# automl/TransformersCanDoBayesianInference

Hardware: NVIDIA H100
Metric: prior-sampled sequences/sec, full training step (prior sample + fwd + bwd + allreduce + clip + Adam) (higher is better)
Workload: dtype bf16

## Files before the change

### transformerscandobayesianinference_b200/csrc/attention_bwd_tc.cu

```cuda
#include "attention_common.cuh"

namespace pfn {

constexpr int AB_ROWS = 64;
constexpr int AB_TILE = AB_ROWS * ATT_ROW_BYTES;
constexpr int AB_THREADS = 3 * 128;
constexpr int AB_DQ_STAGES = 4;
constexpr int AB_DKV_STAGES = 3;
constexpr int AB_DQ_OFF_RING = 4 * AB_TILE;
constexpr int AB_DQ_OFF_BAR = AB_DQ_OFF_RING + AB_DQ_STAGES * 2 * AB_TILE;
constexpr int AB_DQ_SMEM = AB_DQ_OFF_BAR + (2 * AB_DQ_STAGES + 2) * 8 + 1024;
constexpr int AB_DKV_OFF_RING = 4 * AB_TILE;
constexpr int AB_DKV_OFF_STAT = AB_DKV_OFF_RING + AB_DKV_STAGES * 2 * AB_TILE;
constexpr int AB_DKV_OFF_BAR = AB_DKV_OFF_STAT + AB_DKV_STAGES * 2 * AB_ROWS * 4;
constexpr int AB_DKV_SMEM = AB_DKV_OFF_BAR + (2 * AB_DKV_STAGES + 1) * 8 + 1024;
static_assert(AB_DQ_SMEM <= 232448 && AB_DKV_SMEM <= 232448, "the tiles and rings must fit the 227 KB of shared memory");

struct AttnBwdParams {
  int T, B, H, sep;
  float scale, scale_log2;
  const __nv_bfloat16* qkv; int ld_qkv;
  const __nv_bfloat16* dout; int ld_dout;
  __nv_bfloat16* dqkv; int ld_dqkv;
  const float* lse;
  const float* delta;
  int delta_tm;
  float* dq_colsum;
  uint32_t drop_seed; int drop_thr;
  int n_tiles;
  int batch_major;
};

__device__ __forceinline__ float ab_delta(const AttnBwdParams& p, int b, int h, int i) {
  return p.delta_tm ? p.delta[att_tok(i, b, p.T, p.B, 0) * p.H + h] : p.delta[(static_cast<size_t>(b) * p.H + h) * p.T + i];
}

__device__ __forceinline__ uint64_t ab_desc_k(uint32_t tile, int kk) {
  return tc::wgmma_smem_desc(tile + (kk >> 2) * 8192 + (kk & 3) * 32, 16, 1024);
}
__device__ __forceinline__ uint64_t ab_desc_mn(uint32_t tile, int kk) {
  return tc::wgmma_smem_desc(tile + kk * 2048, 8192, 1024);
}
__device__ __forceinline__ uint32_t ab_opaque(uint32_t addr) {
  asm volatile("" : "+r"(addr));
  return addr;
}
__device__ __forceinline__ void ab_mma_n64(float (&d)[32], uint64_t a_desc, uint64_t b_desc, int kk) {
  if (kk == 0) tc::wgmma_m64n64k16<0>(d, a_desc, b_desc);
  else tc::wgmma_m64n64k16<1>(d, a_desc, b_desc);
}

__device__ __forceinline__ void ab_load_tile(uint8_t* dst, const CUtensorMap* m, uint64_t* bar, int col0, int b, int t0) {
  tc::tma_load_3d(dst, m, bar, col0, b, t0);
  tc::tma_load_3d(dst + 8192, m, bar, col0 + 64, b, t0);
}

__global__ void __launch_bounds__(256)
attn_bwd_delta_kernel(const __nv_bfloat16* __restrict__ out, int ld_out, const __nv_bfloat16* __restrict__ dout,
                      int ld_dout, float* __restrict__ delta, int T, int B, int H, int batch_major) {
  const int lane = threadIdx.x & 31;
  const long long warp = (static_cast<long long>(blockIdx.x) * blockDim.x + threadIdx.x) >> 5;
  const long long nwarps = (static_cast<long long>(gridDim.x) * blockDim.x) >> 5;
  const long long rows = static_cast<long long>(T) * B;
  for (long long tok = warp; tok < rows; tok += nwarps) {
    const int t = batch_major ? static_cast<int>(tok % T) : static_cast<int>(tok / B);
    const int b = batch_major ? static_cast<int>(tok / T) : static_cast<int>(tok % B);
    for (int h0 = 0; h0 < H; h0 += 2) {
      const int h = h0 + (lane >> 4);
      float acc = 0.f;
      if (h < H) {
        const int col = h * ATT_DH + (lane & 15) * 8;
        const uint4 pa = *reinterpret_cast<const uint4*>(out + tok * ld_out + col);
        const uint4 pb = *reinterpret_cast<const uint4*>(dout + tok * ld_dout + col);
        const __nv_bfloat162* ha = reinterpret_cast<const __nv_bfloat162*>(&pa);
        const __nv_bfloat162* hb = reinterpret_cast<const __nv_bfloat162*>(&pb);
#pragma unroll
        for (int j = 0; j < 4; ++j) {
// ... 337 lines not shown
    tc::wgmma_commit();
    tc::wgmma_wait<0>();
    if (tid == 0) tc::mbar_arrive(&empty[stage]);
    if (++stage == AB_DKV_STAGES) { stage = 0; phase ^= 1; }
  }
  tc::wgmma_fence_regs(dk);
  tc::wgmma_fence_regs(dv);

#pragma unroll
  for (int r = 0; r < 2; ++r) {
    const int key = key_a + 8 * r;
    if (key < p.sep) {
      __nv_bfloat16* grow = p.dqkv + att_tok(key, b, p.T, p.B, p.batch_major) * p.ld_dqkv + h * ATT_DH;
#pragma unroll
      for (int j = 0; j < 16; ++j) {
        att_st2(grow + E, j, lane, dk[4 * j + 2 * r], dk[4 * j + 2 * r + 1]);
        att_st2(grow + 2 * E, j, lane, dv[4 * j + 2 * r], dv[4 * j + 2 * r + 1]);
      }
    }
  }
  if (timed_out) asm volatile("trap;");
}

static int ab_tensor_map(CUtensorMap* m, const void* base, int cols, int ld, int T, int B, int t_extent, int batch_major) {
  const uint64_t row = static_cast<uint64_t>(ld) * 2;
  const uint64_t dims[3] = {static_cast<uint64_t>(cols), static_cast<uint64_t>(B), static_cast<uint64_t>(t_extent)};
  const uint64_t strides[3] = {0, batch_major ? row * T : row, batch_major ? row : row * B};
  const uint32_t box[3] = {64, 1, AB_ROWS};
  return make_tensor_map(m, base, false, 3, dims, strides, box, true);
}

}

using namespace pfn;

extern "C" int pfn_attention_bwd_tc(const pfn_attn_desc* d, void* stream) {
  if (int rc = check_tc_attn(d, true, "attention_bwd_tc")) return rc;
  PFN_CHECK_ARG(!(d->delta_token_major && d->batch_major), "attention_bwd_tc: a token-major delta implies the reference token order");
  AttnBwdParams p;
  p.T = d->T; p.B = d->B; p.H = d->H; p.sep = d->sep;
  p.scale = d->scale; p.scale_log2 = d->scale * 1.4426950408889634f;
  p.qkv = reinterpret_cast<const __nv_bfloat16*>(d->qkv); p.ld_qkv = d->ld_qkv;
  p.dout = reinterpret_cast<const __nv_bfloat16*>(d->dout); p.ld_dout = d->ld_dout;
  p.dqkv = reinterpret_cast<__nv_bfloat16*>(d->dqkv); p.ld_dqkv = d->ld_dqkv;
  p.lse = d->lse; p.delta = d->delta; p.dq_colsum = d->dq_colsum; p.delta_tm = d->delta_token_major;
  p.drop_seed = d->drop_seed; p.drop_thr = d->drop_thr;
  p.batch_major = d->batch_major;
  const int E = d->H * ATT_DH;
  CUtensorMap tmQ, tmKV, tmDO;
  if (int rc = ab_tensor_map(&tmQ, d->qkv, 3 * E, d->ld_qkv, d->T, d->B, d->T, d->batch_major)) return rc;
  if (int rc = ab_tensor_map(&tmKV, d->qkv, 3 * E, d->ld_qkv, d->T, d->B, d->sep > 0 ? d->sep : 1, d->batch_major)) return rc;
  if (int rc = ab_tensor_map(&tmDO, d->dout, E, d->ld_dout, d->T, d->B, d->T, d->batch_major)) return rc;
  static bool attr_set[64] = {};
  if (first_use_on_device(attr_set)) {
// ... 27 lines not shown
```

### transformerscandobayesianinference_b200/csrc/attention_common.cuh

```cuda
#pragma once
#include "common.cuh"
#include "dropout.cuh"
#include "tc_common.cuh"
#include "../../include/pfn_b200.h"

namespace pfn {

constexpr int ATT_DH = 128;
constexpr int ATT_ROW_BYTES = ATT_DH * 2;

int check_attn_desc_public(const pfn_attn_desc* d, bool bwd, const char* who);

__device__ __forceinline__ uint32_t att_sw(int r, int c) {
  return static_cast<uint32_t>(r * ATT_ROW_BYTES + ((((c >> 3) ^ (r & 7))) << 4) + (c & 7) * 2);
}

__device__ __forceinline__ size_t att_tok(int t, int b, int T, int B, int batch_major) {
  return batch_major ? static_cast<size_t>(b) * T + t : static_cast<size_t>(t) * B + b;
}

template <int NROWS>
__device__ __forceinline__ void att_load_tile(uint8_t* tile, const __nv_bfloat16* base, int ld, int col0, int t0, int t_end,
                                              int b, int T, int B, int batch_major) {
  const uint32_t s = tc::smem_u32(tile);
#pragma unroll
  for (int k = 0; k < NROWS * 16 / 128; ++k) {
    const int idx = static_cast<int>(threadIdx.x) + 128 * k;
    const int r = idx >> 4, c = idx & 15;
    const int t = t0 + r;
    const bool ok = t < t_end;
    const __nv_bfloat16* src = ok ? base + att_tok(t, b, T, B, batch_major) * ld + col0 + c * 8 : base;
    tc::cp_async16(s + att_sw(r, c * 8), src, ok ? 16u : 0u);
  }
}

__device__ __forceinline__ void att_frag_a(uint32_t (&a)[4], uint32_t tile, int r0, int c0, int lane) {
  tc::ldmatrix_x4(a, tile + att_sw(r0 + (lane & 15), c0 + ((lane >> 4) << 3)));
}
__device__ __forceinline__ void att_frag_b(uint32_t (&b)[4], uint32_t tile, int n0, int k0, int lane) {
  tc::ldmatrix_x4(b, tile + att_sw(n0 + (lane & 7) + ((lane >> 4) << 3), k0 + (((lane >> 3) & 1) << 3)));
}
__device__ __forceinline__ void att_frag_bt(uint32_t (&b)[4], uint32_t tile, int k0, int n0, int lane) {
  tc::ldmatrix_x4_trans(b, tile + att_sw(k0 + (lane & 7) + (((lane >> 3) & 1) << 3), n0 + ((lane >> 4) << 3)));
}

__device__ __forceinline__ float2 att_ld2(const __nv_bfloat16* row, int j, int lane) {
  return __bfloat1622float2(*reinterpret_cast<const __nv_bfloat162*>(row + 8 * j + 2 * (lane & 3)));
}
__device__ __forceinline__ void att_st2(__nv_bfloat16* row, int j, int lane, float x, float y) {
  *reinterpret_cast<uint32_t*>(row + 8 * j + 2 * (lane & 3)) = tc::pack_bf16x2(x, y);
}
__device__ __forceinline__ float quad_sum(float v) {
  v += __shfl_xor_sync(0xffffffffu, v, 1);
  return v + __shfl_xor_sync(0xffffffffu, v, 2);
}
__device__ __forceinline__ float quad_max(float v) {
  v = fmaxf(v, __shfl_xor_sync(0xffffffffu, v, 1));
  return fmaxf(v, __shfl_xor_sync(0xffffffffu, v, 2));
}

static inline int check_tc_attn(const pfn_attn_desc* d, bool bwd, const char* who) {
  if (int rc = check_attn_desc_public(d, bwd, who)) return rc;
  PFN_CHECK_ARG(d->dtype == PFN_BF16, "%s: bf16 only", who);
  PFN_CHECK_ARG(d->dh == ATT_DH, "%s: head dim %d unsupported (built for 128)", who, d->dh);
  PFN_CHECK_ARG(d->ld_qkv % 8 == 0 && d->ld_out % 8 == 0, "%s: leading dims must be multiples of 8", who);
  PFN_CHECK_ARG(((reinterpret_cast<uintptr_t>(d->qkv) | reinterpret_cast<uintptr_t>(d->out)) & 15) == 0,
                "%s: qkv/out must be 16-byte aligned", who);
  if (bwd) {
    PFN_CHECK_ARG(d->ld_dout % 8 == 0 && d->ld_dqkv % 8 == 0, "%s: leading dims must be multiples of 8", who);
    PFN_CHECK_ARG(((reinterpret_cast<uintptr_t>(d->dout) | reinterpret_cast<uintptr_t>(d->dqkv)) & 15) == 0,
                  "%s: dout/dqkv must be 16-byte aligned", who);
  }
  return 0;
}

}
```

### transformerscandobayesianinference_b200/csrc/attention_tc.cu

```cuda
#include "attention_common.cuh"

namespace pfn {

constexpr int ATT_BM = 64;
constexpr int ATT_BN = 64;
constexpr int ATT_TILE_BYTES = ATT_BM * ATT_ROW_BYTES;
constexpr int ATT_FWD_SMEM = 5 * ATT_TILE_BYTES;

struct AttnFwdParams {
  int T, B, H, sep;
  float scale_log2;
  const __nv_bfloat16* qkv; int ld_qkv;
  __nv_bfloat16* out; int ld_out;
  float* lse;
  int n_qtiles;
  int batch_major;
  uint32_t drop_seed; int drop_thr;
};

__global__ void __launch_bounds__(128, 2)
attn_fwd_tc_kernel(const AttnFwdParams p) {
  extern __shared__ __align__(128) uint8_t smem[];
  uint8_t* sQ = smem;
  uint8_t* sK = smem + ATT_TILE_BYTES;
  uint8_t* sV = smem + 3 * ATT_TILE_BYTES;
  const int warp = threadIdx.x >> 5, lane = threadIdx.x & 31;
  const int qt = static_cast<int>(blockIdx.x) % p.n_qtiles;
  const int bh = static_cast<int>(blockIdx.x) / p.n_qtiles;
  const int h = bh % p.H, b = bh / p.H;
  const int E = p.H * ATT_DH;
  const int i0 = qt * ATT_BM;
  const int nblk = (p.sep + ATT_BN - 1) / ATT_BN;

  att_load_tile<ATT_BM>(sQ, p.qkv, p.ld_qkv, h * ATT_DH, i0, p.T, b, p.T, p.B, p.batch_major);
  if (nblk > 0) {
    att_load_tile<ATT_BN>(sK, p.qkv, p.ld_qkv, E + h * ATT_DH, 0, p.sep, b, p.T, p.B, p.batch_major);
    att_load_tile<ATT_BN>(sV, p.qkv, p.ld_qkv, 2 * E + h * ATT_DH, 0, p.sep, b, p.T, p.B, p.batch_major);
  }
  tc::cp_async_commit();

  float o[16][4];
#pragma unroll
  for (int j = 0; j < 16; ++j) o[j][0] = o[j][1] = o[j][2] = o[j][3] = 0.f;
  float m[2] = {-INFINITY, -INFINITY}, l[2] = {0.f, 0.f};
  const int r0 = 16 * warp;
  const uint32_t drow0 = static_cast<uint32_t>(bh) * p.T + i0 + r0 + (lane >> 2);
  const uint32_t q_s = tc::smem_u32(sQ);

  for (int kb = 0; kb < nblk; ++kb) {
    if (kb + 1 < nblk) {
      const int nb = (kb + 1) & 1;
      att_load_tile<ATT_BN>(sK + nb * ATT_TILE_BYTES, p.qkv, p.ld_qkv, E + h * ATT_DH, (kb + 1) * ATT_BN, p.sep, b, p.T, p.B, p.batch_major);
      att_load_tile<ATT_BN>(sV + nb * ATT_TILE_BYTES, p.qkv, p.ld_qkv, 2 * E + h * ATT_DH, (kb + 1) * ATT_BN, p.sep, b, p.T, p.B, p.batch_major);
      tc::cp_async_commit();
      tc::cp_async_wait<1>();
    } else {
      tc::cp_async_wait<0>();
    }
    __syncthreads();
    const uint32_t k_s = tc::smem_u32(sK + (kb & 1) * ATT_TILE_BYTES);
    const uint32_t v_s = tc::smem_u32(sV + (kb & 1) * ATT_TILE_BYTES);

    float s[8][4];
#pragma unroll
    for (int j = 0; j < 8; ++j) s[j][0] = s[j][1] = s[j][2] = s[j][3] = 0.f;
#pragma unroll
    for (int kk = 0; kk < 8; ++kk) {
      uint32_t a[4];
      att_frag_a(a, q_s, r0, kk * 16, lane);
#pragma unroll
      for (int np = 0; np < 4; ++np) {
        uint32_t bb[4];
        att_frag_b(bb, k_s, np * 16, kk * 16, lane);
        tc::mma_bf16_16816(s[2 * np], a, bb[0], bb[1]);
        tc::mma_bf16_16816(s[2 * np + 1], a, bb[2], bb[3]);
      }
    }
    const int key0 = kb * ATT_BN + 2 * (lane & 3);
    float mx[2] = {-INFINITY, -INFINITY};
#pragma unroll
    for (int j = 0; j < 8; ++j)
#pragma unroll
      for (int e = 0; e < 4; ++e) {
        const bool ok = key0 + 8 * j + (e & 1) < p.sep;
        s[j][e] = ok ? s[j][e] * p.scale_log2 : -INFINITY;
        mx[e >> 1] = fmaxf(mx[e >> 1], s[j][e]);
      }
    float corr[2];
#pragma unroll
    for (int r = 0; r < 2; ++r) {
      const float mn = fmaxf(m[r], quad_max(mx[r]));
      corr[r] = fast_ex2(m[r] - mn);
      m[r] = mn;
      l[r] *= corr[r];
    }
#pragma unroll
    for (int j = 0; j < 8; ++j)
#pragma unroll
      for (int e = 0; e < 4; ++e) {
        const float pr = fast_ex2(s[j][e] - m[e >> 1]);
        l[e >> 1] += pr;
        if (p.drop_thr > 0 && !drop_keep(p.drop_seed, drow0 + 8 * (e >> 1), key0 + 8 * j + (e & 1), p.drop_thr)) s[j][e] = 0.f;
        else s[j][e] = pr;
      }
#pragma unroll
    for (int j = 0; j < 16; ++j) {
      o[j][0] *= corr[0]; o[j][1] *= corr[0];
      o[j][2] *= corr[1]; o[j][3] *= corr[1];
    }
#pragma unroll
    for (int kk = 0; kk < 4; ++kk) {
      uint32_t a[4];
      a[0] = tc::pack_bf16x2(s[2 * kk][0], s[2 * kk][1]);
      a[1] = tc::pack_bf16x2(s[2 * kk][2], s[2 * kk][3]);
      a[2] = tc::pack_bf16x2(s[2 * kk + 1][0], s[2 * kk + 1][1]);
      a[3] = tc::pack_bf16x2(s[2 * kk + 1][2], s[2 * kk + 1][3]);
#pragma unroll
      for (int dp = 0; dp < 8; ++dp) {
        uint32_t bb[4];
        att_frag_bt(bb, v_s, kk * 16, dp * 16, lane);
        tc::mma_bf16_16816(o[2 * dp], a, bb[0], bb[1]);
        tc::mma_bf16_16816(o[2 * dp + 1], a, bb[2], bb[3]);
      }
    }
    __syncthreads();
  }

  const float dscale = p.drop_thr > 0 ? drop_scale(p.drop_thr) : 1.0f;
#pragma unroll
  for (int r = 0; r < 2; ++r) {
    const int i = i0 + r0 + (lane >> 2) + 8 * r;
    float lr = quad_sum(l[r]);
    const bool valid = i < p.T;
    const bool diag = valid && i >= p.sep;
    const __nv_bfloat16* qrow = p.qkv + att_tok(valid ? i : 0, b, p.T, p.B, p.batch_major) * p.ld_qkv + h * ATT_DH;
    float sd = 0.f;
    if (diag) {
#pragma unroll
      for (int j = 0; j < 16; ++j) {
        const float2 q = att_ld2(qrow, j, lane), k = att_ld2(qrow + E, j, lane);
        sd = fmaf(q.x, k.x, fmaf(q.y, k.y, sd));
      }
    }
    sd = quad_sum(sd) * p.scale_log2;
    if (diag) {
      const float mn = fmaxf(m[r], sd);
      const float c = fast_ex2(m[r] - mn);
      const float pr = fast_ex2(sd - mn);
      lr = lr * c + pr;
      m[r] = mn;
      const float pd = (p.drop_thr > 0 && !drop_keep(p.drop_seed, drow0 + 8 * r, i, p.drop_thr)) ? 0.f : pr;
#pragma unroll
      for (int j = 0; j < 16; ++j) {
        const float2 v = att_ld2(qrow + 2 * E, j, lane);
        o[j][2 * r] = fmaf(pd, v.x, o[j][2 * r] * c);
        o[j][2 * r + 1] = fmaf(pd, v.y, o[j][2 * r + 1] * c);
      }
    }
    if (valid) {
      const float inv = dscale / lr;
      __nv_bfloat16* orow = p.out + att_tok(i, b, p.T, p.B, p.batch_major) * p.ld_out + h * ATT_DH;
#pragma unroll
      for (int j = 0; j < 16; ++j) att_st2(orow, j, lane, o[j][2 * r] * inv, o[j][2 * r + 1] * inv);
      if ((lane & 3) == 0) p.lse[static_cast<size_t>(bh) * p.T + i] = (m[r] + __log2f(lr)) * 0.69314718055994531f;
    }
  }
}

}

using namespace pfn;

extern "C" int pfn_attention_fwd_tc(const pfn_attn_desc* d, void* stream) {
  if (int rc = check_tc_attn(d, false, "attention_fwd_tc")) return rc;
  AttnFwdParams p;
  p.T = d->T; p.B = d->B; p.H = d->H; p.sep = d->sep;
  p.scale_log2 = d->scale * 1.4426950408889634f;
  p.qkv = reinterpret_cast<const __nv_bfloat16*>(d->qkv); p.ld_qkv = d->ld_qkv;
  p.out = reinterpret_cast<__nv_bfloat16*>(d->out); p.ld_out = d->ld_out;
  p.lse = d->lse;
  p.n_qtiles = (d->T + ATT_BM - 1) / ATT_BM;
  p.batch_major = d->batch_major;
  p.drop_seed = d->drop_seed; p.drop_thr = d->drop_thr;
  const long long grid = static_cast<long long>(p.n_qtiles) * d->B * d->H;
  PFN_CHECK_ARG(grid < (1LL << 31), "attention_fwd_tc: too many tiles");
  static bool attr_set[64] = {};
  if (first_use_on_device(attr_set)) {
    PFN_CUDA_OK(cudaFuncSetAttribute(attn_fwd_tc_kernel, cudaFuncAttributeMaxDynamicSharedMemorySize, ATT_FWD_SMEM));
  }
  attn_fwd_tc_kernel<<<static_cast<unsigned>(grid), 128, ATT_FWD_SMEM, reinterpret_cast<cudaStream_t>(stream)>>>(p);
  PFN_LAUNCH_OK();
  return 0;
}
```

### transformerscandobayesianinference_b200/csrc/tc_common.cuh

```cuda
#pragma once
#include <cuda.h>
#include <cuda_bf16.h>
#include <cuda_runtime.h>
#include <stdint.h>

namespace pfn {
namespace tc {

__device__ __forceinline__ uint32_t smem_u32(const void* p) {
  return static_cast<uint32_t>(__cvta_generic_to_shared(p));
}

__device__ __forceinline__ void mbar_init(uint64_t* bar, uint32_t count) {
  asm volatile("mbarrier.init.shared::cta.b64 [%0], %1;" ::"r"(smem_u32(bar)), "r"(count) : "memory");
}
__device__ __forceinline__ void mbar_fence_init() {
  asm volatile("fence.mbarrier_init.release.cluster;" ::: "memory");
}
__device__ __forceinline__ void mbar_expect_tx(uint64_t* bar, uint32_t bytes) {
  asm volatile("mbarrier.arrive.expect_tx.shared::cta.b64 _, [%0], %1;" ::"r"(smem_u32(bar)), "r"(bytes) : "memory");
}
__device__ __forceinline__ void mbar_arrive(uint64_t* bar) {
  asm volatile("mbarrier.arrive.shared::cta.b64 _, [%0];" ::"r"(smem_u32(bar)) : "memory");
}
// ... 39 lines not shown
    if (++spins > PFN_MBAR_SPIN_LIMIT) asm volatile("trap;");
  }
}
__device__ __forceinline__ void tma_prefetch_desc(const CUtensorMap* m) {
  asm volatile("prefetch.tensormap [%0];" ::"l"(reinterpret_cast<uint64_t>(m)) : "memory");
}
__device__ __forceinline__ void tma_load_2d(void* smem_dst, const CUtensorMap* m, uint64_t* bar, int c0, int c1) {
  asm volatile(
      "cp.async.bulk.tensor.2d.shared::cluster.global.tile.mbarrier::complete_tx::bytes [%0], [%1, {%3, %4}], [%2];"
      ::"r"(smem_u32(smem_dst)), "l"(reinterpret_cast<uint64_t>(m)), "r"(smem_u32(bar)), "r"(c0), "r"(c1)
      : "memory");
}
__device__ __forceinline__ void tma_load_3d(void* smem_dst, const CUtensorMap* m, uint64_t* bar, int c0, int c1, int c2) {
  asm volatile(
      "cp.async.bulk.tensor.3d.shared::cluster.global.tile.mbarrier::complete_tx::bytes [%0], [%1, {%3, %4, %5}], [%2];"
      ::"r"(smem_u32(smem_dst)), "l"(reinterpret_cast<uint64_t>(m)), "r"(smem_u32(bar)), "r"(c0), "r"(c1), "r"(c2)
      : "memory");
}
__device__ __forceinline__ void tma_store_2d(const CUtensorMap* m, const void* smem_src, int c0, int c1) {
  asm volatile("cp.async.bulk.tensor.2d.global.shared::cta.tile.bulk_group [%0, {%2, %3}], [%1];"
               ::"l"(reinterpret_cast<uint64_t>(m)), "r"(smem_u32(smem_src)), "r"(c0), "r"(c1)
               : "memory");
}
__device__ __forceinline__ void tma_reduce_add_2d(const CUtensorMap* m, const void* smem_src, int c0, int c1) {
  asm volatile("cp.reduce.async.bulk.tensor.2d.global.shared::cta.add.tile.bulk_group [%0, {%2, %3}], [%1];"
               ::"l"(reinterpret_cast<uint64_t>(m)), "r"(smem_u32(smem_src)), "r"(c0), "r"(c1)
               : "memory");
}
__device__ __forceinline__ void bulk_commit() { asm volatile("cp.async.bulk.commit_group;" ::: "memory"); }
template <int N>
__device__ __forceinline__ void bulk_wait_read() {
  asm volatile("cp.async.bulk.wait_group.read %0;" ::"n"(N) : "memory");
}
template <int N>
__device__ __forceinline__ void bulk_wait() {
  asm volatile("cp.async.bulk.wait_group %0;" ::"n"(N) : "memory");
}
__device__ __forceinline__ void fence_proxy_async_smem() { asm volatile("fence.proxy.async.shared::cta;" ::: "memory"); }

__device__ __forceinline__ void named_bar_sync(int id, int threads) {
  asm volatile("bar.sync %0, %1;" ::"r"(id), "r"(threads) : "memory");
}
__device__ __forceinline__ void named_bar_arrive(int id, int threads) {
  asm volatile("bar.arrive %0, %1;" ::"r"(id), "r"(threads) : "memory");
}
template <int N>
// ... 1 lines not shown
template <int N>
__device__ __forceinline__ void setmaxnreg_inc() { asm volatile("setmaxnreg.inc.sync.aligned.u32 %0;" ::"n"(N)); }

__device__ __forceinline__ uint32_t pack_bf16x2(float lo, float hi) {
  __nv_bfloat162 t = __floats2bfloat162_rn(lo, hi);
  return *reinterpret_cast<uint32_t*>(&t);
}

__device__ __forceinline__ uint64_t wgmma_smem_desc(uint32_t smem_addr, uint32_t lbo_bytes, uint32_t sbo_bytes) {
  return (1ull << 62) | (static_cast<uint64_t>((sbo_bytes >> 4) & 0x3FFF) << 32) |
         (static_cast<uint64_t>((lbo_bytes >> 4) & 0x3FFF) << 16) | static_cast<uint64_t>((smem_addr >> 4) & 0x3FFF);
}

__device__ __forceinline__ void wgmma_fence() { asm volatile("wgmma.fence.sync.aligned;" ::: "memory"); }
__device__ __forceinline__ void wgmma_commit() { asm volatile("wgmma.commit_group.sync.aligned;" ::: "memory"); }
template <int N>
__device__ __forceinline__ void wgmma_wait() {
  asm volatile("wgmma.wait_group.sync.aligned %0;" ::"n"(N) : "memory");
}
template <int N>
__device__ __forceinline__ void wgmma_fence_regs(float (&d)[N]) {
#pragma unroll
  for (int i = 0; i < N; ++i) asm volatile("" : "+f"(d[i])::"memory");
}

template <int TA, int TB>
__device__ __forceinline__ void wgmma_m64n128k16(float (&d)[64], uint64_t a_desc, uint64_t b_desc, uint32_t accumulate) {
  asm volatile(
      "{\n\t.reg .pred p;\n\t"
      "setp.ne.b32 p, %66, 0;\n\t"
      "wgmma.mma_async.sync.aligned.m64n128k16.f32.bf16.bf16 "
      "{%0, %1, %2, %3, %4, %5, %6, %7, %8, %9, %10, %11, %12, %13, %14, %15, "
      "%16, %17, %18, %19, %20, %21, %22, %23, %24, %25, %26, %27, %28, %29, %30, %31, "
      "%32, %33, %34, %35, %36, %37, %38, %39, %40, %41, %42, %43, %44, %45, %46, %47, "
      "%48, %49, %50, %51, %52, %53, %54, %55, %56, %57, %58, %59, %60, %61, %62, %63}, "
      "%64, %65, p, 1, 1, %67, %68;\n\t}"
      : "+f"(d[0]), "+f"(d[1]), "+f"(d[2]), "+f"(d[3]), "+f"(d[4]), "+f"(d[5]), "+f"(d[6]), "+f"(d[7]),
        "+f"(d[8]), "+f"(d[9]), "+f"(d[10]), "+f"(d[11]), "+f"(d[12]), "+f"(d[13]), "+f"(d[14]), "+f"(d[15]),
        "+f"(d[16]), "+f"(d[17]), "+f"(d[18]), "+f"(d[19]), "+f"(d[20]), "+f"(d[21]), "+f"(d[22]), "+f"(d[23]),
        "+f"(d[24]), "+f"(d[25]), "+f"(d[26]), "+f"(d[27]), "+f"(d[28]), "+f"(d[29]), "+f"(d[30]), "+f"(d[31]),
        "+f"(d[32]), "+f"(d[33]), "+f"(d[34]), "+f"(d[35]), "+f"(d[36]), "+f"(d[37]), "+f"(d[38]), "+f"(d[39]),
        "+f"(d[40]), "+f"(d[41]), "+f"(d[42]), "+f"(d[43]), "+f"(d[44]), "+f"(d[45]), "+f"(d[46]), "+f"(d[47]),
        "+f"(d[48]), "+f"(d[49]), "+f"(d[50]), "+f"(d[51]), "+f"(d[52]), "+f"(d[53]), "+f"(d[54]), "+f"(d[55]),
        "+f"(d[56]), "+f"(d[57]), "+f"(d[58]), "+f"(d[59]), "+f"(d[60]), "+f"(d[61]), "+f"(d[62]), "+f"(d[63])
      : "l"(a_desc), "l"(b_desc), "r"(accumulate), "n"(TA), "n"(TB));
}
// ... 18 lines not shown
#undef PFN_WGMMA_D32

__device__ __forceinline__ void wgmma_m64n128k16_rs(float (&d)[64], const uint32_t* a, uint64_t b_desc, uint32_t accumulate) {
  asm volatile(
      "{\n\t.reg .pred p;\n\t"
      "setp.ne.b32 p, %69, 0;\n\t"
      "wgmma.mma_async.sync.aligned.m64n128k16.f32.bf16.bf16 "
      "{%0, %1, %2, %3, %4, %5, %6, %7, %8, %9, %10, %11, %12, %13, %14, %15, "
      "%16, %17, %18, %19, %20, %21, %22, %23, %24, %25, %26, %27, %28, %29, %30, %31, "
      "%32, %33, %34, %35, %36, %37, %38, %39, %40, %41, %42, %43, %44, %45, %46, %47, "
      "%48, %49, %50, %51, %52, %53, %54, %55, %56, %57, %58, %59, %60, %61, %62, %63}, "
      "{%64, %65, %66, %67}, %68, p, 1, 1, 1;\n\t}"
      : "+f"(d[0]), "+f"(d[1]), "+f"(d[2]), "+f"(d[3]), "+f"(d[4]), "+f"(d[5]), "+f"(d[6]), "+f"(d[7]),
        "+f"(d[8]), "+f"(d[9]), "+f"(d[10]), "+f"(d[11]), "+f"(d[12]), "+f"(d[13]), "+f"(d[14]), "+f"(d[15]),
        "+f"(d[16]), "+f"(d[17]), "+f"(d[18]), "+f"(d[19]), "+f"(d[20]), "+f"(d[21]), "+f"(d[22]), "+f"(d[23]),
        "+f"(d[24]), "+f"(d[25]), "+f"(d[26]), "+f"(d[27]), "+f"(d[28]), "+f"(d[29]), "+f"(d[30]), "+f"(d[31]),
        "+f"(d[32]), "+f"(d[33]), "+f"(d[34]), "+f"(d[35]), "+f"(d[36]), "+f"(d[37]), "+f"(d[38]), "+f"(d[39]),
        "+f"(d[40]), "+f"(d[41]), "+f"(d[42]), "+f"(d[43]), "+f"(d[44]), "+f"(d[45]), "+f"(d[46]), "+f"(d[47]),
        "+f"(d[48]), "+f"(d[49]), "+f"(d[50]), "+f"(d[51]), "+f"(d[52]), "+f"(d[53]), "+f"(d[54]), "+f"(d[55]),
        "+f"(d[56]), "+f"(d[57]), "+f"(d[58]), "+f"(d[59]), "+f"(d[60]), "+f"(d[61]), "+f"(d[62]), "+f"(d[63])
      : "r"(a[0]), "r"(a[1]), "r"(a[2]), "r"(a[3]), "l"(b_desc), "r"(accumulate));
}

__device__ __forceinline__ void mma_bf16_16816(float (&c)[4], const uint32_t (&a)[4], uint32_t b0, uint32_t b1) {
  asm volatile(
      "mma.sync.aligned.m16n8k16.row.col.f32.bf16.bf16.f32 {%0, %1, %2, %3}, {%4, %5, %6, %7}, {%8, %9}, "
      "{%0, %1, %2, %3};"
      : "+f"(c[0]), "+f"(c[1]), "+f"(c[2]), "+f"(c[3])
      : "r"(a[0]), "r"(a[1]), "r"(a[2]), "r"(a[3]), "r"(b0), "r"(b1));
}
__device__ __forceinline__ void ldmatrix_x4(uint32_t (&r)[4], uint32_t addr) {
  asm volatile("ldmatrix.sync.aligned.m8n8.x4.shared.b16 {%0, %1, %2, %3}, [%4];"
               : "=r"(r[0]), "=r"(r[1]), "=r"(r[2]), "=r"(r[3])
               : "r"(addr));
}
__device__ __forceinline__ void ldmatrix_x4_trans(uint32_t (&r)[4], uint32_t addr) {
  asm volatile("ldmatrix.sync.aligned.m8n8.x4.trans.shared.b16 {%0, %1, %2, %3}, [%4];"
               : "=r"(r[0]), "=r"(r[1]), "=r"(r[2]), "=r"(r[3])
               : "r"(addr));
}
__device__ __forceinline__ void cp_async16(uint32_t dst, const void* src, uint32_t src_bytes) {
  asm volatile("cp.async.cg.shared.global [%0], [%1], 16, %2;" ::"r"(dst), "l"(src), "r"(src_bytes) : "memory");
}
__device__ __forceinline__ void cp_async_commit() { asm volatile("cp.async.commit_group;" ::: "memory"); }
template <int N>
__device__ __forceinline__ void cp_async_wait() {
  asm volatile("cp.async.wait_group %0;" ::"n"(N) : "memory");
}

}

int make_tensor_map(CUtensorMap* out, const void* base, bool f32, int rank, const uint64_t* dims,
                    const uint64_t* strides_bytes, const uint32_t* box, bool swizzle128);

}
```

Measured before the change: 2327.

## Rewrite attention forward as persistent warp-specialized WGMMA kernel with TMA pipeline

Replaces the mma.sync/cp.async forward attention kernel with a persistent kernel. A producer warpgroup streams K/V tiles through a 3-stage mbarrier ring using TMA, and two consumer warpgroups each process 64 query rows with WGMMA. The diagonal self-attention term is computed up front from TMA-loaded tiles rather than from extra global reads at the end. Output is staged in shared memory and written with TMA stores. This is meant to raise tensor-core utilization and overlap loads with compute, at the cost of much more complex synchronization, register reallocation and a bounded-wait trap path.

```diff
diff --git a/transformerscandobayesianinference_b200/csrc/attention_bwd_tc.cu b/transformerscandobayesianinference_b200/csrc/attention_bwd_tc.cu
--- a/transformerscandobayesianinference_b200/csrc/attention_bwd_tc.cu
+++ b/transformerscandobayesianinference_b200/csrc/attention_bwd_tc.cu
@@ -2,9 +2,6 @@
 
 namespace pfn {
 
-constexpr int AB_ROWS = 64;
-constexpr int AB_TILE = AB_ROWS * ATT_ROW_BYTES;
-constexpr int AB_THREADS = 3 * 128;
 constexpr int AB_DQ_STAGES = 4;
 constexpr int AB_DKV_STAGES = 3;
 constexpr int AB_DQ_OFF_RING = 4 * AB_TILE;
@@ -33,26 +30,6 @@
 
 __device__ __forceinline__ float ab_delta(const AttnBwdParams& p, int b, int h, int i) {
   return p.delta_tm ? p.delta[att_tok(i, b, p.T, p.B, 0) * p.H + h] : p.delta[(static_cast<size_t>(b) * p.H + h) * p.T + i];
-}
-
-__device__ __forceinline__ uint64_t ab_desc_k(uint32_t tile, int kk) {
-  return tc::wgmma_smem_desc(tile + (kk >> 2) * 8192 + (kk & 3) * 32, 16, 1024);
-}
-__device__ __forceinline__ uint64_t ab_desc_mn(uint32_t tile, int kk) {
-  return tc::wgmma_smem_desc(tile + kk * 2048, 8192, 1024);
-}
-__device__ __forceinline__ uint32_t ab_opaque(uint32_t addr) {
-  asm volatile("" : "+r"(addr));
-  return addr;
-}
-__device__ __forceinline__ void ab_mma_n64(float (&d)[32], uint64_t a_desc, uint64_t b_desc, int kk) {
-  if (kk == 0) tc::wgmma_m64n64k16<0>(d, a_desc, b_desc);
-  else tc::wgmma_m64n64k16<1>(d, a_desc, b_desc);
-}
-
-__device__ __forceinline__ void ab_load_tile(uint8_t* dst, const CUtensorMap* m, uint64_t* bar, int col0, int b, int t0) {
-  tc::tma_load_3d(dst, m, bar, col0, b, t0);
-  tc::tma_load_3d(dst + 8192, m, bar, col0 + 64, b, t0);
 }
 
 __global__ void __launch_bounds__(256)
@@ -436,14 +413,6 @@
   if (timed_out) asm volatile("trap;");
 }
 
-static int ab_tensor_map(CUtensorMap* m, const void* base, int cols, int ld, int T, int B, int t_extent, int batch_major) {
-  const uint64_t row = static_cast<uint64_t>(ld) * 2;
-  const uint64_t dims[3] = {static_cast<uint64_t>(cols), static_cast<uint64_t>(B), static_cast<uint64_t>(t_extent)};
-  const uint64_t strides[3] = {0, batch_major ? row * T : row, batch_major ? row : row * B};
-  const uint32_t box[3] = {64, 1, AB_ROWS};
-  return make_tensor_map(m, base, false, 3, dims, strides, box, true);
-}
-
 }
 
 using namespace pfn;
diff --git a/transformerscandobayesianinference_b200/csrc/attention_common.cuh b/transformerscandobayesianinference_b200/csrc/attention_common.cuh
--- a/transformerscandobayesianinference_b200/csrc/attention_common.cuh
+++ b/transformerscandobayesianinference_b200/csrc/attention_common.cuh
@@ -11,37 +11,42 @@
 
 int check_attn_desc_public(const pfn_attn_desc* d, bool bwd, const char* who);
 
-__device__ __forceinline__ uint32_t att_sw(int r, int c) {
-  return static_cast<uint32_t>(r * ATT_ROW_BYTES + ((((c >> 3) ^ (r & 7))) << 4) + (c & 7) * 2);
-}
-
 __device__ __forceinline__ size_t att_tok(int t, int b, int T, int B, int batch_major) {
   return batch_major ? static_cast<size_t>(b) * T + t : static_cast<size_t>(t) * B + b;
 }
 
-template <int NROWS>
-__device__ __forceinline__ void att_load_tile(uint8_t* tile, const __nv_bfloat16* base, int ld, int col0, int t0, int t_end,
-                                              int b, int T, int B, int batch_major) {
-  const uint32_t s = tc::smem_u32(tile);
-#pragma unroll
-  for (int k = 0; k < NROWS * 16 / 128; ++k) {
-    const int idx = static_cast<int>(threadIdx.x) + 128 * k;
-    const int r = idx >> 4, c = idx & 15;
-    const int t = t0 + r;
-    const bool ok = t < t_end;
-    const __nv_bfloat16* src = ok ? base + att_tok(t, b, T, B, batch_major) * ld + col0 + c * 8 : base;
-    tc::cp_async16(s + att_sw(r, c * 8), src, ok ? 16u : 0u);
-  }
+constexpr int AB_ROWS = 64;
+constexpr int AB_TILE = AB_ROWS * ATT_ROW_BYTES;
+constexpr int AB_THREADS = 3 * 128;
+
+__device__ __forceinline__ uint64_t ab_desc_k(uint32_t tile, int kk) {
+  return tc::wgmma_smem_desc(tile + (kk >> 2) * 8192 + (kk & 3) * 32, 16, 1024);
+}
+__device__ __forceinline__ uint64_t ab_desc_mn(uint32_t tile, int kk) {
+  return tc::wgmma_smem_desc(tile + kk * 2048, 8192, 1024);
+}
+__device__ __forceinline__ uint32_t ab_opaque(uint32_t addr) {
+  asm volatile("" : "+r"(addr));
+  return addr;
+}
+__device__ __forceinline__ void ab_mma_n64(float (&d)[32], uint64_t a_desc, uint64_t b_desc, int kk) {
+  if (kk == 0) tc::wgmma_m64n64k16<0>(d, a_desc, b_desc);
+  else tc::wgmma_m64n64k16<1>(d, a_desc, b_desc);
 }
 
-__device__ __forceinline__ void att_frag_a(uint32_t (&a)[4], uint32_t tile, int r0, int c0, int lane) {
-  tc::ldmatrix_x4(a, tile + att_sw(r0 + (lane & 15), c0 + ((lane >> 4) << 3)));
+__device__ __forceinline__ void ab_load_tile(uint8_t* dst, const CUtensorMap* m, uint64_t* bar, int col0, int b, int t0) {
+  tc::tma_load_3d(dst, m, bar, col0, b, t0);
+  tc::tma_load_3d(dst + 8192, m, bar, col0 + 64, b, t0);
 }
-__device__ __forceinline__ void att_frag_b(uint32_t (&b)[4], uint32_t tile, int n0, int k0, int lane) {
-  tc::ldmatrix_x4(b, tile + att_sw(n0 + (lane & 7) + ((lane >> 4) << 3), k0 + (((lane >> 3) & 1) << 3)));
+
+__device__ __forceinline__ uint32_t ab_sw(int r, int j, int lane) {
+  return static_cast<uint32_t>((j >> 3) * 8192 + r * 128 + (((j & 7) ^ (r & 7)) << 4) + 4 * (lane & 3));
 }
-__device__ __forceinline__ void att_frag_bt(uint32_t (&b)[4], uint32_t tile, int k0, int n0, int lane) {
-  tc::ldmatrix_x4_trans(b, tile + att_sw(k0 + (lane & 7) + (((lane >> 3) & 1) << 3), n0 + ((lane >> 4) << 3)));
+__device__ __forceinline__ float2 ab_ld2(const uint8_t* tile, int r, int j, int lane) {
+  return __bfloat1622float2(*reinterpret_cast<const __nv_bfloat162*>(tile + ab_sw(r, j, lane)));
+}
+__device__ __forceinline__ void ab_st2(uint8_t* tile, int r, int j, int lane, float x, float y) {
+  *reinterpret_cast<uint32_t*>(tile + ab_sw(r, j, lane)) = tc::pack_bf16x2(x, y);
 }
 
 __device__ __forceinline__ float2 att_ld2(const __nv_bfloat16* row, int j, int lane) {
@@ -57,6 +62,14 @@
 __device__ __forceinline__ float quad_max(float v) {
   v = fmaxf(v, __shfl_xor_sync(0xffffffffu, v, 1));
   return fmaxf(v, __shfl_xor_sync(0xffffffffu, v, 2));
+}
+
+static inline int ab_tensor_map(CUtensorMap* m, const void* base, int cols, int ld, int T, int B, int t_extent, int batch_major) {
+  const uint64_t row = static_cast<uint64_t>(ld) * 2;
+  const uint64_t dims[3] = {static_cast<uint64_t>(cols), static_cast<uint64_t>(B), static_cast<uint64_t>(t_extent)};
+  const uint64_t strides[3] = {0, batch_major ? row * T : row, batch_major ? row : row * B};
+  const uint32_t box[3] = {64, 1, AB_ROWS};
+  return make_tensor_map(m, base, false, 3, dims, strides, box, true);
 }
 
 static inline int check_tc_attn(const pfn_attn_desc* d, bool bwd, const char* who) {
diff --git a/transformerscandobayesianinference_b200/csrc/attention_tc.cu b/transformerscandobayesianinference_b200/csrc/attention_tc.cu
--- a/transformerscandobayesianinference_b200/csrc/attention_tc.cu
+++ b/transformerscandobayesianinference_b200/csrc/attention_tc.cu
@@ -2,169 +2,254 @@
 
 namespace pfn {
 
-constexpr int ATT_BM = 64;
-constexpr int ATT_BN = 64;
-constexpr int ATT_TILE_BYTES = ATT_BM * ATT_ROW_BYTES;
-constexpr int ATT_FWD_SMEM = 5 * ATT_TILE_BYTES;
+constexpr int AF_STAGES = 3;
+constexpr int AF_OFF_KD = 2 * AB_TILE;
+constexpr int AF_OFF_VD = 4 * AB_TILE;
+constexpr int AF_OFF_O = 6 * AB_TILE;
+constexpr int AF_OFF_RING = 8 * AB_TILE;
+constexpr int AF_OFF_BAR = AF_OFF_RING + AF_STAGES * 2 * AB_TILE;
+constexpr int AF_SMEM = AF_OFF_BAR + (2 * AF_STAGES + 2) * 8 + 1024;
+static_assert(AF_SMEM <= 232448, "the tiles and the ring must fit the 227 KB of shared memory");
 
 struct AttnFwdParams {
   int T, B, H, sep;
   float scale_log2;
-  const __nv_bfloat16* qkv; int ld_qkv;
-  __nv_bfloat16* out; int ld_out;
   float* lse;
-  int n_qtiles;
-  int batch_major;
+  int n_tiles;
   uint32_t drop_seed; int drop_thr;
 };
 
-__global__ void __launch_bounds__(128, 2)
-attn_fwd_tc_kernel(const AttnFwdParams p) {
-  extern __shared__ __align__(128) uint8_t smem[];
+__device__ __forceinline__ bool af_has_diag(const AttnFwdParams& p, int qt, int g) {
+  return qt * 128 + 64 * g < p.T && min(p.T, qt * 128 + 64 * g + 64) > p.sep;
+}
+
+__global__ void __launch_bounds__(AB_THREADS, 1)
+attn_fwd_tc_kernel(const __grid_constant__ CUtensorMap tmQ, const __grid_constant__ CUtensorMap tmKV,
+                   const __grid_constant__ CUtensorMap tmO, const AttnFwdParams p) {
+  extern __shared__ uint8_t smem_raw[];
+  uint8_t* smem = smem_raw + ((1024u - (tc::smem_u32(smem_raw) & 1023u)) & 1023u);
   uint8_t* sQ = smem;
-  uint8_t* sK = smem + ATT_TILE_BYTES;
-  uint8_t* sV = smem + 3 * ATT_TILE_BYTES;
+  uint8_t* sKd = smem + AF_OFF_KD;
+  uint8_t* sVd = smem + AF_OFF_VD;
+  uint8_t* sO = smem + AF_OFF_O;
+  uint8_t* sRing = smem + AF_OFF_RING;
+  uint64_t* kv_full = reinterpret_cast<uint64_t*>(smem + AF_OFF_BAR);
+  uint64_t* kv_empty = kv_full + AF_STAGES;
+  uint64_t* q_full = kv_empty + AF_STAGES;
+  uint64_t* q_empty = q_full + 1;
   const int warp = threadIdx.x >> 5, lane = threadIdx.x & 31;
-  const int qt = static_cast<int>(blockIdx.x) % p.n_qtiles;
-  const int bh = static_cast<int>(blockIdx.x) / p.n_qtiles;
-  const int h = bh % p.H, b = bh / p.H;
   const int E = p.H * ATT_DH;
-  const int i0 = qt * ATT_BM;
-  const int nblk = (p.sep + ATT_BN - 1) / ATT_BN;
-
-  att_load_tile<ATT_BM>(sQ, p.qkv, p.ld_qkv, h * ATT_DH, i0, p.T, b, p.T, p.B, p.batch_major);
-  if (nblk > 0) {
-    att_load_tile<ATT_BN>(sK, p.qkv, p.ld_qkv, E + h * ATT_DH, 0, p.sep, b, p.T, p.B, p.batch_major);
-    att_load_tile<ATT_BN>(sV, p.qkv, p.ld_qkv, 2 * E + h * ATT_DH, 0, p.sep, b, p.T, p.B, p.batch_major);
-  }
-  tc::cp_async_commit();
-
-  float o[16][4];
-#pragma unroll
-  for (int j = 0; j < 16; ++j) o[j][0] = o[j][1] = o[j][2] = o[j][3] = 0.f;
-  float m[2] = {-INFINITY, -INFINITY}, l[2] = {0.f, 0.f};
-  const int r0 = 16 * warp;
-  const uint32_t drow0 = static_cast<uint32_t>(bh) * p.T + i0 + r0 + (lane >> 2);
-  const uint32_t q_s = tc::smem_u32(sQ);
-
-  for (int kb = 0; kb < nblk; ++kb) {
-    if (kb + 1 < nblk) {
-      const int nb = (kb + 1) & 1;
-      att_load_tile<ATT_BN>(sK + nb * ATT_TILE_BYTES, p.qkv, p.ld_qkv, E + h * ATT_DH, (kb + 1) * ATT_BN, p.sep, b, p.T, p.B, p.batch_major);
-      att_load_tile<ATT_BN>(sV + nb * ATT_TILE_BYTES, p.qkv, p.ld_qkv, 2 * E + h * ATT_DH, (kb + 1) * ATT_BN, p.sep, b, p.T, p.B, p.batch_major);
-      tc::cp_async_commit();
-      tc::cp_async_wait<1>();
+  const int nblk = (p.sep + AB_ROWS - 1) / AB_ROWS;
+  const int n_units = p.n_tiles * p.B * p.H;
+  if (threadIdx.x == 0) {
+    for (int s = 0; s < AF_STAGES; ++s) {
+      tc::mbar_init(&kv_full[s], 1);
+      tc::mbar_init(&kv_empty[s], 2);
+    }
+    tc::mbar_init(q_full, 1);
+    tc::mbar_init(q_empty, 2);
+    tc::mbar_fence_init();
+  }
+  __syncthreads();
+
+  if (warp >= 8) {
+    tc::setmaxnreg_dec<40>();
+    if (threadIdx.x == 256) {
+      tc::tma_prefetch_desc(&tmQ);
+      tc::tma_prefetch_desc(&tmKV);
+      tc::tma_prefetch_desc(&tmO);
+      int stage = 0;
+      uint32_t phase = 0;
+      for (int u = blockIdx.x, it = 0; u < n_units; u += gridDim.x, ++it) {
+        const int qt = u % p.n_tiles, bh = u / p.n_tiles;
+        const int h = bh % p.H, b = bh / p.H;
+        auto load_q = [&]() {
+          if (it > 0) tc::mbar_wait_suspend(q_empty, (it - 1) & 1);
+          const bool d0 = af_has_diag(p, qt, 0), d1 = af_has_diag(p, qt, 1);
+          tc::mbar_expect_tx(q_full, (2 + 2 * d0 + 2 * d1) * AB_TILE);
+          for (int g = 0; g < 2; ++g) {
+            const int t0 = qt * 128 + 64 * g;
+            ab_load_tile(sQ + g * AB_TILE, &tmQ, q_full, h * ATT_DH, b, t0);
+            if (g == 0 ? d0 : d1) {
+              ab_load_tile(sKd + g * AB_TILE, &tmQ, q_full, E + h * ATT_DH, b, t0);
+              ab_load_tile(sVd + g * AB_TILE, &tmQ, q_full, 2 * E + h * ATT_DH, b, t0);
+            }
+          }
+        };
+        const int claim_at = min(AF_STAGES - 1, nblk - 1);
+        if (nblk == 0) load_q();
+        for (int kb = 0; kb < nblk; ++kb) {
+          if (kb == claim_at) load_q();
+          tc::mbar_wait_suspend(&kv_empty[stage], phase ^ 1);
+          uint8_t* dst = sRing + stage * 2 * AB_TILE;
+          tc::mbar_expect_tx(&kv_full[stage], 2 * AB_TILE);
+          ab_load_tile(dst, &tmKV, &kv_full[stage], E + h * ATT_DH, b, kb * AB_ROWS);
+          ab_load_tile(dst + AB_TILE, &tmKV, &kv_full[stage], 2 * E + h * ATT_DH, b, kb * AB_ROWS);
+          if (++stage == AF_STAGES) { stage = 0; phase ^= 1; }
+        }
+      }
+    }
+    return;
+  }
+
+  tc::setmaxnreg_inc<232>();
+  const int g = warp >> 2, wq = warp & 3;
+  const int tid = threadIdx.x & 127;
+  const int rr = 16 * wq + (lane >> 2);
+  const uint32_t q_tile = tc::smem_u32(sQ + g * AB_TILE);
+  const uint8_t* kd = sKd + g * AB_TILE;
+  const uint8_t* vd = sVd + g * AB_TILE;
+  uint8_t* so = sO + g * AB_TILE;
+  const float dscale = p.drop_thr > 0 ? drop_scale(p.drop_thr) : 1.0f;
+  int stage = 0;
+  uint32_t phase = 0;
+  bool timed_out = false;
+  for (int u = blockIdx.x, it = 0; u < n_units && !timed_out; u += gridDim.x, ++it) {
+    const int qt = u % p.n_tiles, bh = u / p.n_tiles;
+    const int h = bh % p.H, b = bh / p.H;
+    const int i0 = qt * 128 + 64 * g + rr;
+    const uint32_t drow0 = static_cast<uint32_t>(bh) * p.T + i0;
+    if (!tc::mbar_wait_bounded(q_full, it & 1)) { timed_out = true; break; }
+
+    float o[64], m[2], l[2];
+#pragma unroll
+    for (int r = 0; r < 2; ++r) {
+      const int i = i0 + 8 * r;
+      const bool diag = i >= p.sep && i < p.T;
+      const uint8_t* qs = sQ + g * AB_TILE;
+      float sd = 0.f;
+      if (diag) {
+#pragma unroll
+        for (int j = 0; j < 16; ++j) {
+          const float2 q = ab_ld2(qs, rr + 8 * r, j, lane), k = ab_ld2(kd, rr + 8 * r, j, lane);
+          sd = fmaf(q.x, k.x, fmaf(q.y, k.y, sd));
+        }
+      }
+      sd = quad_sum(sd) * p.scale_log2;
+      m[r] = diag ? sd : -INFINITY;
+      l[r] = diag && (lane & 3) == 0 ? 1.f : 0.f;
+      const float pd = diag && !(p.drop_thr > 0 && !drop_keep(p.drop_seed, drow0 + 8 * r, i, p.drop_thr)) ? 1.f : 0.f;
+#pragma unroll
+      for (int j = 0; j < 16; ++j) {
+        const float2 v = diag ? ab_ld2(vd, rr + 8 * r, j, lane) : make_float2(0.f, 0.f);
+        o[4 * j + 2 * r] = pd * v.x;
+        o[4 * j + 2 * r + 1] = pd * v.y;
+      }
+    }
+
+    auto softmax = [&](const float (&s)[32], int kb, float (&corr)[2], uint32_t (&pb)[16]) {
+      const int key0 = kb * AB_ROWS + 2 * (lane & 3);
+      auto scaled = [&](int j, int e) { return key0 + 8 * j + (e & 1) < p.sep ? s[4 * j + e] * p.scale_log2 : -INFINITY; };
+      float mx[2] = {-INFINITY, -INFINITY};
+#pragma unroll
+      for (int j = 0; j < 8; ++j)
+#pragma unroll
+        for (int e = 0; e < 4; ++e) mx[e >> 1] = fmaxf(mx[e >> 1], scaled(j, e));
+#pragma unroll
+      for (int r = 0; r < 2; ++r) {
+        const float mn = fmaxf(m[r], quad_max(mx[r]));
+        corr[r] = fast_ex2(m[r] - mn);
+        m[r] = mn;
+        l[r] *= corr[r];
+      }
+#pragma unroll
+      for (int j = 0; j < 8; ++j)
+#pragma unroll
+        for (int e = 0; e < 4; e += 2) {
+          float pr[2];
+#pragma unroll
+          for (int c = 0; c < 2; ++c) {
+            pr[c] = fast_ex2(scaled(j, e + c) - m[e >> 1]);
+            l[e >> 1] += pr[c];
+            if (p.drop_thr > 0 && !drop_keep(p.drop_seed, drow0 + 8 * (e >> 1), key0 + 8 * j + c, p.drop_thr)) pr[c] = 0.f;
+          }
+          pb[2 * j + (e >> 1)] = tc::pack_bf16x2(pr[0], pr[1]);
+        }
+    };
+    auto rescale = [&](const float (&corr)[2]) {
+#pragma unroll
+      for (int j = 0; j < 16; ++j) {
+        o[4 * j] *= corr[0]; o[4 * j + 1] *= corr[0];
+        o[4 * j + 2] *= corr[1]; o[4 * j + 3] *= corr[1];
+      }
+    };
+
+    if (nblk == 0) {
+      if (tid == 0) tc::mbar_arrive(q_empty);
     } else {
-      tc::cp_async_wait<0>();
-    }
-    __syncthreads();
-    const uint32_t k_s = tc::smem_u32(sK + (kb & 1) * ATT_TILE_BYTES);
-    const uint32_t v_s = tc::smem_u32(sV + (kb & 1) * ATT_TILE_BYTES);
-
-    float s[8][4];
-#pragma unroll
-    for (int j = 0; j < 8; ++j) s[j][0] = s[j][1] = s[j][2] = s[j][3] = 0.f;
-#pragma unroll
-    for (int kk = 0; kk < 8; ++kk) {
-      uint32_t a[4];
-      att_frag_a(a, q_s, r0, kk * 16, lane);
-#pragma unroll
-      for (int np = 0; np < 4; ++np) {
-        uint32_t bb[4];
-        att_frag_b(bb, k_s, np * 16, kk * 16, lane);
-        tc::mma_bf16_16816(s[2 * np], a, bb[0], bb[1]);
-        tc::mma_bf16_16816(s[2 * np + 1], a, bb[2], bb[3]);
-      }
-    }
-    const int key0 = kb * ATT_BN + 2 * (lane & 3);
-    float mx[2] = {-INFINITY, -INFINITY};
-#pragma unroll
-    for (int j = 0; j < 8; ++j)
-#pragma unroll
-      for (int e = 0; e < 4; ++e) {
-        const bool ok = key0 + 8 * j + (e & 1) < p.sep;
-        s[j][e] = ok ? s[j][e] * p.scale_log2 : -INFINITY;
-        mx[e >> 1] = fmaxf(mx[e >> 1], s[j][e]);
-      }
-    float corr[2];
+      float s[32], corr[2];
+      uint32_t pa[16], pb[16];
+      if (!tc::mbar_wait_bounded(&kv_full[stage], phase)) { timed_out = true; break; }
+      {
+        const uint32_t q_s = ab_opaque(q_tile), k_s = tc::smem_u32(sRing + stage * 2 * AB_TILE);
+        tc::wgmma_fence();
+#pragma unroll
+        for (int kk = 0; kk < 8; ++kk) ab_mma_n64(s, ab_desc_k(q_s, kk), ab_desc_k(k_s, kk), kk);
+        tc::wgmma_commit();
+        tc::wgmma_wait<0>();
+        tc::wgmma_fence_regs(s);
+      }
+      if (nblk == 1 && tid == 0) tc::mbar_arrive(q_empty);
+      softmax(s, 0, corr, pa);
+      rescale(corr);
+      for (int kb = 0; kb < nblk; ++kb) {
+        const int cur = stage;
+        const uint32_t v_s = tc::smem_u32(sRing + cur * 2 * AB_TILE) + AB_TILE;
+        if (++stage == AF_STAGES) { stage = 0; phase ^= 1; }
+        const bool more = kb + 1 < nblk;
+        if (more && !tc::mbar_wait_bounded(&kv_full[stage], phase)) { timed_out = true; break; }
+        tc::wgmma_fence();
+        if (more) {
+          const uint32_t q_s = ab_opaque(q_tile), k_s = tc::smem_u32(sRing + stage * 2 * AB_TILE);
+#pragma unroll
+          for (int kk = 0; kk < 8; ++kk) ab_mma_n64(s, ab_desc_k(q_s, kk), ab_desc_k(k_s, kk), kk);
+          tc::wgmma_commit();
+        }
+#pragma unroll
+        for (int kk = 0; kk < 4; ++kk) tc::wgmma_m64n128k16_rs(o, pa + 4 * kk, ab_desc_mn(v_s, kk), 1);
+        tc::wgmma_commit();
+        if (more) {
+          tc::wgmma_wait<1>();
+          tc::wgmma_fence_regs(s);
+          if (kb + 2 == nblk && tid == 0) tc::mbar_arrive(q_empty);
+          softmax(s, kb + 1, corr, pb);
+          tc::wgmma_wait<0>();
+          tc::wgmma_fence_regs(o);
+          tc::wgmma_fence_regs(pa);
+          if (tid == 0) tc::mbar_arrive(&kv_empty[cur]);
+          rescale(corr);
+#pragma unroll
+          for (int k = 0; k < 16; ++k) pa[k] = pb[k];
+        } else {
+          tc::wgmma_wait<0>();
+          tc::wgmma_fence_regs(o);
+          if (tid == 0) tc::mbar_arrive(&kv_empty[cur]);
+        }
+      }
+      if (timed_out) break;
+    }
+
+    if (tid == 0) tc::bulk_wait_read<0>();
+    tc::named_bar_sync(1 + g, 128);
 #pragma unroll
     for (int r = 0; r < 2; ++r) {
-      const float mn = fmaxf(m[r], quad_max(mx[r]));
-      corr[r] = fast_ex2(m[r] - mn);
-      m[r] = mn;
-      l[r] *= corr[r];
-    }
-#pragma unroll
-    for (int j = 0; j < 8; ++j)
-#pragma unroll
-      for (int e = 0; e < 4; ++e) {
-        const float pr = fast_ex2(s[j][e] - m[e >> 1]);
-        l[e >> 1] += pr;
-        if (p.drop_thr > 0 && !drop_keep(p.drop_seed, drow0 + 8 * (e >> 1), key0 + 8 * j + (e & 1), p.drop_thr)) s[j][e] = 0.f;
-        else s[j][e] = pr;
-      }
-#pragma unroll
-    for (int j = 0; j < 16; ++j) {
-      o[j][0] *= corr[0]; o[j][1] *= corr[0];
-      o[j][2] *= corr[1]; o[j][3] *= corr[1];
-    }
-#pragma unroll
-    for (int kk = 0; kk < 4; ++kk) {
-      uint32_t a[4];
-      a[0] = tc::pack_bf16x2(s[2 * kk][0], s[2 * kk][1]);
-      a[1] = tc::pack_bf16x2(s[2 * kk][2], s[2 * kk][3]);
-      a[2] = tc::pack_bf16x2(s[2 * kk + 1][0], s[2 * kk + 1][1]);
-      a[3] = tc::pack_bf16x2(s[2 * kk + 1][2], s[2 * kk + 1][3]);
-#pragma unroll
-      for (int dp = 0; dp < 8; ++dp) {
-        uint32_t bb[4];
-        att_frag_bt(bb, v_s, kk * 16, dp * 16, lane);
-        tc::mma_bf16_16816(o[2 * dp], a, bb[0], bb[1]);
-        tc::mma_bf16_16816(o[2 * dp + 1], a, bb[2], bb[3]);
-      }
-    }
-    __syncthreads();
-  }
-
-  const float dscale = p.drop_thr > 0 ? drop_scale(p.drop_thr) : 1.0f;
-#pragma unroll
-  for (int r = 0; r < 2; ++r) {
-    const int i = i0 + r0 + (lane >> 2) + 8 * r;
-    float lr = quad_sum(l[r]);
-    const bool valid = i < p.T;
-    const bool diag = valid && i >= p.sep;
-    const __nv_bfloat16* qrow = p.qkv + att_tok(valid ? i : 0, b, p.T, p.B, p.batch_major) * p.ld_qkv + h * ATT_DH;
-    float sd = 0.f;
-    if (diag) {
-#pragma unroll
-      for (int j = 0; j < 16; ++j) {
-        const float2 q = att_ld2(qrow, j, lane), k = att_ld2(qrow + E, j, lane);
-        sd = fmaf(q.x, k.x, fmaf(q.y, k.y, sd));
-      }
-    }
-    sd = quad_sum(sd) * p.scale_log2;
-    if (diag) {
-      const float mn = fmaxf(m[r], sd);
-      const float c = fast_ex2(m[r] - mn);
-      const float pr = fast_ex2(sd - mn);
-      lr = lr * c + pr;
-      m[r] = mn;
-      const float pd = (p.drop_thr > 0 && !drop_keep(p.drop_seed, drow0 + 8 * r, i, p.drop_thr)) ? 0.f : pr;
-#pragma unroll
-      for (int j = 0; j < 16; ++j) {
-        const float2 v = att_ld2(qrow + 2 * E, j, lane);
-        o[j][2 * r] = fmaf(pd, v.x, o[j][2 * r] * c);
-        o[j][2 * r + 1] = fmaf(pd, v.y, o[j][2 * r + 1] * c);
-      }
-    }
-    if (valid) {
+      const int i = i0 + 8 * r;
+      const float lr = quad_sum(l[r]);
       const float inv = dscale / lr;
-      __nv_bfloat16* orow = p.out + att_tok(i, b, p.T, p.B, p.batch_major) * p.ld_out + h * ATT_DH;
-#pragma unroll
-      for (int j = 0; j < 16; ++j) att_st2(orow, j, lane, o[j][2 * r] * inv, o[j][2 * r + 1] * inv);
-      if ((lane & 3) == 0) p.lse[static_cast<size_t>(bh) * p.T + i] = (m[r] + __log2f(lr)) * 0.69314718055994531f;
-    }
-  }
+#pragma unroll
+      for (int j = 0; j < 16; ++j) ab_st2(so, rr + 8 * r, j, lane, o[4 * j + 2 * r] * inv, o[4 * j + 2 * r + 1] * inv);
+      if (i < p.T && (lane & 3) == 0) p.lse[static_cast<size_t>(bh) * p.T + i] = (m[r] + __log2f(lr)) * 0.69314718055994531f;
+    }
+    tc::fence_proxy_async_smem();
+    tc::named_bar_sync(1 + g, 128);
+    if (tid == 0) {
+      tc::tma_store_3d(&tmO, so, h * ATT_DH, b, qt * 128 + 64 * g);
+      tc::tma_store_3d(&tmO, so + 8192, h * ATT_DH + 64, b, qt * 128 + 64 * g);
+      tc::bulk_commit();
+    }
+  }
+  if (tid == 0) tc::bulk_wait<0>();
+  if (timed_out) asm volatile("trap;");
 }
 
 }
@@ -176,19 +261,22 @@
   AttnFwdParams p;
   p.T = d->T; p.B = d->B; p.H = d->H; p.sep = d->sep;
   p.scale_log2 = d->scale * 1.4426950408889634f;
-  p.qkv = reinterpret_cast<const __nv_bfloat16*>(d->qkv); p.ld_qkv = d->ld_qkv;
-  p.out = reinterpret_cast<__nv_bfloat16*>(d->out); p.ld_out = d->ld_out;
   p.lse = d->lse;
-  p.n_qtiles = (d->T + ATT_BM - 1) / ATT_BM;
-  p.batch_major = d->batch_major;
+  p.n_tiles = (d->T + 127) / 128;
   p.drop_seed = d->drop_seed; p.drop_thr = d->drop_thr;
-  const long long grid = static_cast<long long>(p.n_qtiles) * d->B * d->H;
-  PFN_CHECK_ARG(grid < (1LL << 31), "attention_fwd_tc: too many tiles");
+  const long long units = static_cast<long long>(p.n_tiles) * d->B * d->H;
+  PFN_CHECK_ARG(units < (1LL << 31), "attention_fwd_tc: too many tiles");
+  const int E = d->H * ATT_DH;
+  CUtensorMap tmQ, tmKV, tmO;
+  if (int rc = ab_tensor_map(&tmQ, d->qkv, 3 * E, d->ld_qkv, d->T, d->B, d->T, d->batch_major)) return rc;
+  if (int rc = ab_tensor_map(&tmKV, d->qkv, 3 * E, d->ld_qkv, d->T, d->B, d->sep > 0 ? d->sep : 1, d->batch_major)) return rc;
+  if (int rc = ab_tensor_map(&tmO, d->out, E, d->ld_out, d->T, d->B, d->T, d->batch_major)) return rc;
   static bool attr_set[64] = {};
   if (first_use_on_device(attr_set)) {
-    PFN_CUDA_OK(cudaFuncSetAttribute(attn_fwd_tc_kernel, cudaFuncAttributeMaxDynamicSharedMemorySize, ATT_FWD_SMEM));
-  }
-  attn_fwd_tc_kernel<<<static_cast<unsigned>(grid), 128, ATT_FWD_SMEM, reinterpret_cast<cudaStream_t>(stream)>>>(p);
+    PFN_CUDA_OK(cudaFuncSetAttribute(attn_fwd_tc_kernel, cudaFuncAttributeMaxDynamicSharedMemorySize, AF_SMEM));
+  }
+  const int grid = units < num_sms() ? static_cast<int>(units) : num_sms();
+  attn_fwd_tc_kernel<<<static_cast<unsigned>(grid), AB_THREADS, AF_SMEM, reinterpret_cast<cudaStream_t>(stream)>>>(tmQ, tmKV, tmO, p);
   PFN_LAUNCH_OK();
   return 0;
 }
diff --git a/transformerscandobayesianinference_b200/csrc/tc_common.cuh b/transformerscandobayesianinference_b200/csrc/tc_common.cuh
--- a/transformerscandobayesianinference_b200/csrc/tc_common.cuh
+++ b/transformerscandobayesianinference_b200/csrc/tc_common.cuh
@@ -85,6 +85,11 @@
                ::"l"(reinterpret_cast<uint64_t>(m)), "r"(smem_u32(smem_src)), "r"(c0), "r"(c1)
                : "memory");
 }
+__device__ __forceinline__ void tma_store_3d(const CUtensorMap* m, const void* smem_src, int c0, int c1, int c2) {
+  asm volatile("cp.async.bulk.tensor.3d.global.shared::cta.tile.bulk_group [%0, {%2, %3, %4}], [%1];"
+               ::"l"(reinterpret_cast<uint64_t>(m)), "r"(smem_u32(smem_src)), "r"(c0), "r"(c1), "r"(c2)
+               : "memory");
+}
 __device__ __forceinline__ void tma_reduce_add_2d(const CUtensorMap* m, const void* smem_src, int c0, int c1) {
   asm volatile("cp.reduce.async.bulk.tensor.2d.global.shared::cta.add.tile.bulk_group [%0, {%2, %3}], [%1];"
                ::"l"(reinterpret_cast<uint64_t>(m)), "r"(smem_u32(smem_src)), "r"(c0), "r"(c1)
@@ -132,6 +137,11 @@
 __device__ __forceinline__ void wgmma_fence_regs(float (&d)[N]) {
 #pragma unroll
   for (int i = 0; i < N; ++i) asm volatile("" : "+f"(d[i])::"memory");
+}
+template <int N>
+__device__ __forceinline__ void wgmma_fence_regs(uint32_t (&a)[N]) {
+#pragma unroll
+  for (int i = 0; i < N; ++i) asm volatile("" : "+r"(a[i])::"memory");
 }
 
 template <int TA, int TB>
@@ -196,32 +206,6 @@
       : "r"(a[0]), "r"(a[1]), "r"(a[2]), "r"(a[3]), "l"(b_desc), "r"(accumulate));
 }
 
-__device__ __forceinline__ void mma_bf16_16816(float (&c)[4], const uint32_t (&a)[4], uint32_t b0, uint32_t b1) {
-  asm volatile(
-      "mma.sync.aligned.m16n8k16.row.col.f32.bf16.bf16.f32 {%0, %1, %2, %3}, {%4, %5, %6, %7}, {%8, %9}, "
-      "{%0, %1, %2, %3};"
-      : "+f"(c[0]), "+f"(c[1]), "+f"(c[2]), "+f"(c[3])
-      : "r"(a[0]), "r"(a[1]), "r"(a[2]), "r"(a[3]), "r"(b0), "r"(b1));
-}
-__device__ __forceinline__ void ldmatrix_x4(uint32_t (&r)[4], uint32_t addr) {
-  asm volatile("ldmatrix.sync.aligned.m8n8.x4.shared.b16 {%0, %1, %2, %3}, [%4];"
-               : "=r"(r[0]), "=r"(r[1]), "=r"(r[2]), "=r"(r[3])
-               : "r"(addr));
-}
-__device__ __forceinline__ void ldmatrix_x4_trans(uint32_t (&r)[4], uint32_t addr) {
-  asm volatile("ldmatrix.sync.aligned.m8n8.x4.trans.shared.b16 {%0, %1, %2, %3}, [%4];"
-               : "=r"(r[0]), "=r"(r[1]), "=r"(r[2]), "=r"(r[3])
-               : "r"(addr));
-}
-__device__ __forceinline__ void cp_async16(uint32_t dst, const void* src, uint32_t src_bytes) {
-  asm volatile("cp.async.cg.shared.global [%0], [%1], 16, %2;" ::"r"(dst), "l"(src), "r"(src_bytes) : "memory");
-}
-__device__ __forceinline__ void cp_async_commit() { asm volatile("cp.async.commit_group;" ::: "memory"); }
-template <int N>
-__device__ __forceinline__ void cp_async_wait() {
-  asm volatile("cp.async.wait_group %0;" ::"n"(N) : "memory");
-}
-
 }
 
 int make_tensor_map(CUtensorMap* out, const void* base, bool f32, int rank, const uint64_t* dims,
```

New measurement: 2409 (median of 6 runs). 3.5% higher.
